# itz-sayak/C-Users-Sayakdutta-Self-Supervised-Arbitrary-Scale-Point-Cloud-Upsampling-via-SNN

Measured on AMD Instinct MI355X. Metric: upsampled query-points/sec (kNN + fn fwd + rotate + fd fwd + displace), 4x scale, M=48 T=4, higher is better.
Workload: dtype f32 (GEMMs as 3 x f16 MFMA with f32 accumulation; outer kNN f64); 1 GPU; synthetic sphere N=5000 (seed 0), B=4096 grid queries per GPU per step, M=48, T=4, fn k=[24,18,12] emb 640, fd k=32 scales [8,16,32,48] emb 768, conditioned-random weights seed 0, in-patch kNN recomputed every batch; cloud_points=5000, neighbours=48, outer_knn=f64 brute force, parallelism=query shards x1

## Files before the change

c-users-sayakdutta-self-supervised-arbitrary-scale-point-cloud-upsampling-via-snn_amd/csrc/common.h:

```cpp
#pragma once
#include <hip/hip_runtime.h>
#include <stdint.h>
#include <stdio.h>
#include <string.h>
#include "../../include/sapcu.h"

namespace sapcu {

void set_error(const char* fmt, ...);

#define SAPCU_CHECK_ARG(cond, ...)                      \
    do {                                                \
        if (!(cond)) {                                  \
            ::sapcu::set_error(__VA_ARGS__);            \
            return SAPCU_ERR_ARG;                       \
        }                                               \
    } while (0)

#define SAPCU_CHECK_HIP(expr)                                                            \
    do {                                                                                 \
        hipError_t _e = (expr);                                                          \
        if (_e != hipSuccess) {                                                          \
            ::sapcu::set_error("%s failed: %s (%s:%d)", #expr, hipGetErrorString(_e),    \
                               __FILE__, __LINE__);                                      \
// ... 134 lines not shown
    g = g * 0.19947114020071633897f;
#else
    const f32x2 a = pk_fma(x * x, f32x2{-0.72134752044448170368f, -0.72134752044448170368f},
                           f32x2{-2.3257480647361593f, -2.3257480647361593f});
    g.x = __builtin_amdgcn_exp2f(a.x);
    g.y = __builtin_amdgcn_exp2f(a.y);
#endif
    e.x = __builtin_amdgcn_exp2f(b.x);
    e.y = __builtin_amdgcn_exp2f(b.y);
    const f32x2 den = e + 1.0f;
    s.x = __builtin_amdgcn_rcpf(den.x);
    s.y = __builtin_amdgcn_rcpf(den.y);
    return pk_fma(f32x2{0.5f, 0.5f}, s, g);
}

template <int H>
__device__ __forceinline__ void lif_selfloop_pairs(f32x2 (&v)[H], const NeuronP2 (&p)[H], int T) {
    f32x2 m[H], r[H], th[H], s[H];
#pragma unroll
    for (int u = 0; u < H; ++u) {
        m[u] = v[u];
        s[u] = soft_spike2(m[u] - p[u].theta0);
    }
    if (T > 1) {
#ifdef SAPCU_LIF_EXACT_ORDER
#pragma unroll
        for (int u = 0; u < H; ++u) {
            m[u] = m[u] * (1.0f - s[u]);
            r[u] = s[u];
            const f32x2 t0 = p[u].theta0 + p[u].adapt * s[u];
            th[u] = p[u].theta0 + (t0 - p[u].theta0) * 0.95f;
        }
// ... 13 lines not shown
        for (int u = 0; u < H; ++u) {
            const f32x2 mm = (m[u] * p[u].decay) * (1.0f - r[u]);
            s[u] = soft_spike2(mm - th[u]);
        }
#else
        f32x2 a95[H], thc[H];
        const f32x2 k95 = f32x2{0.95f, 0.95f};
#pragma unroll
        for (int u = 0; u < H; ++u) {
            a95[u] = p[u].adapt * 0.95f;
            thc[u] = p[u].theta0 * 0.05f;
            m[u] = pk_fma(-m[u], s[u], m[u]);
            r[u] = s[u];
            th[u] = pk_fma(p[u].theta0, k95, pk_fma(s[u], a95[u], thc[u]));
        }
        for (int t = 1; t < T - 1; ++t) {
#pragma unroll
            for (int u = 0; u < H; ++u) {
                const f32x2 md = m[u] * p[u].decay;
                const f32x2 mm = pk_fma(-md, r[u], md);
                const f32x2 sp = soft_spike2(mm - th[u]);
                m[u] = pk_fma(-mm, sp, mm);
                r[u] = pk_fma(r[u], p[u].rdecay, sp);
                th[u] = pk_fma(th[u], k95, pk_fma(sp, a95[u], thc[u]));
                s[u] = sp;
            }
        }
#pragma unroll
        for (int u = 0; u < H; ++u) {
            const f32x2 md = m[u] * p[u].decay;
            s[u] = soft_spike2(pk_fma(-md, r[u], md) - th[u]);
        }
#endif
    }
#pragma unroll
    for (int u = 0; u < H; ++u) v[u] = s[u];
}

template <int W>
__device__ __forceinline__ void lif_selfloop_n(float (&v)[W], const NeuronP& p, int T) {
    constexpr int H = (W + 1) / 2;
    f32x2 pv[H];
    NeuronP2 pp[H];
#pragma unroll
    for (int u = 0; u < H; ++u) {
        pv[u] = f32x2{v[2 * u], v[(2 * u + 1 < W) ? 2 * u + 1 : 2 * u]};
        pp[u] = NeuronP2{{p.decay, p.decay}, {p.adapt, p.adapt}, {p.rdecay, p.rdecay}, {p.theta0, p.theta0}};
    }
    lif_selfloop_pairs<H>(pv, pp, T);
#pragma unroll
    for (int u = 0; u < H; ++u) {
        v[2 * u] = pv[u].x;
        if (2 * u + 1 < W) v[2 * u + 1] = pv[u].y;
    }
}

__device__ __forceinline__ float lif_selfloop(float x, const NeuronP& p, int T) {
    float v[1] = {x};
    lif_selfloop_n<1>(v, p, T);
    return v[0];
}

struct NeuronS2 {
    f32x2 m, th, r;
// ... 208 lines not shown
```

c-users-sayakdutta-self-supervised-arbitrary-scale-point-cloud-upsampling-via-snn_amd/csrc/fn_edge_chain.hip:

```cpp
#include "common.h"
#include "gemm_epi.h"
#include "ops.h"

namespace sapcu {
typedef _Float16 half8 __attribute__((ext_vector_type(8)));

#ifndef SAPCU_CHAIN_LB128
#define SAPCU_CHAIN_LB128 3
#endif
#ifndef SAPCU_CHAIN_FCD_MFMA
#define SAPCU_CHAIN_FCD_MFMA(D) ((D) == 256)
#endif
template <int D> struct ChainShape {
    static constexpr int ROWS = D == 128 ? 96 : (D == 256 ? 128 : 64);
    static constexpr int RS = ROWS / 16;
    static constexpr int CB = D == 512 ? 2 : 1;
    static constexpr int CS = 2 * CB;
    static constexpr int NW = D / (32 * CB);
    static constexpr int PLANE = ROWS * 64;
    static constexpr int KSTEP = 2 * PLANE;
    static constexpr int LDS = ROWS * D * 4 + ROWS * 16 + ROWS * 8;
    static constexpr int US = 8;
};

template <int D, int KK> struct ChainSlots {
    static constexpr int GS = 4 * ChainShape<D>::RS;
// ... 5 lines not shown
        if (t < KK) return g;
        const int p = 4 + (g * SP + t - KK) / KK;
        return p < PPG ? p : -1;
    }
    static constexpr int nbr(int rs, int g, int e) {
        const int t = 4 * rs + e;
        return t < KK ? t : (g * SP + t - KK) % KK;
    }
    static constexpr int SP1 = SP > 0 ? SP : 1;
    static constexpr int ua_g(int n, int jj) { return (n * KK + jj) / SP1; }
    static constexpr int ua_rs(int n, int jj) { return (KK + (n * KK + jj) % SP1) >> 2; }
    static constexpr int ua_e(int n, int jj) { return (KK + (n * KK + jj) % SP1) & 3; }
};

__global__ __launch_bounds__(256) void edge_prep_kernel(const float* __restrict__ patch, const int32_t* __restrict__ idx,
                                                        int64_t rows, int m, int kk, int2* __restrict__ tab,
                                                        float4* __restrict__ pd) {
    const int64_t r = (int64_t)blockIdx.x * blockDim.x + threadIdx.x;
    if (r >= rows) return;
    const int64_t pt = r / kk;
    const int64_t nrow = (pt / m) * m + idx[r];
    tab[r] = make_int2((int)pt, (int)nrow);
    const float* pi = patch + pt * 3;
    const float* pj = patch + nrow * 3;
    pd[r] = make_float4(__fsub_rn(pi[0], pj[0]), __fsub_rn(pi[1], pj[1]), __fsub_rn(pi[2], pj[2]), 0.f);
}

__global__ __launch_bounds__(256) void pack_chain_weights_kernel(const _Float16* __restrict__ hi, const _Float16* __restrict__ lo,
                                                                 int d, _Float16* __restrict__ out) {
    const int64_t t = (int64_t)blockIdx.x * blockDim.x + threadIdx.x;
    const int nk32 = d / 32;
    const int64_t total = (int64_t)(d / 16) * nk32 * 2 * 64;
    if (t >= total) return;
    const int lane = (int)(t & 63);
    const int plane = (int)((t >> 6) & 1);
    const int64_t cs_s = t >> 7;
    const int s = (int)(cs_s % nk32), cs = (int)(cs_s / nk32);
    const _Float16* src = (plane ? lo : hi) + (int64_t)(16 * cs + (lane & 15)) * d + 32 * s + 8 * (lane >> 4);
    *reinterpret_cast<half8*>(out + t * 8) = *reinterpret_cast<const half8*>(src);
}
// ... 224 lines not shown
#pragma unroll
    for (int jj = 0; jj < KK; jj += 2) {
        const f32x2 w2 = f32x2{xs[jj], xs[jj + 1]} * inv2;
        out = __fmaf_rn(w2.x, ts[jj], out);
        out = __fmaf_rn(w2.y, ts[jj + 1], out);
    }
    return out;
}

template <int KK>
__device__ __forceinline__ float chain_softmax_agg(float (&xs)[KK], const float (&ts)[KK]) {
    const float den = chain_softmax_den<KK>(xs);
    return chain_softmax_out<KK>(xs, ts, den);
}

template <int D, int KK, bool O32, bool FILL, bool TRIM>
__device__ __forceinline__ void fn_edge_chain_body(const ChainArgs& a) {
    static_assert(!FILL || (D == 512 && KK == 12), "filled groups: d = 512, kk = 12");
    static_assert(ChainSlots<D, KK>::NUA == 0 || (ChainSlots<D, KK>::NUA == 1 && ChainSlots<D, KK>::SP == 4 && KK == 12) ||
                      (ChainSlots<D, KK>::NUA == 3 && ChainSlots<D, KK>::SP == 14 && KK == 18),
                  "the trimmed spare-slot sums are written for the slot layouts of d = 256 / kk = 18 and d = 512 / kk = 12");
    using S = ChainShape<D>;
    using M = ChainSlots<D, KK>;
    constexpr int CH_ROWS = S::ROWS, RS = S::RS, CS = S::CS, CH_PLANE = S::PLANE, CH_KSTEP = S::KSTEP;
    constexpr int PPG = M::PPG, NUA = M::NUA, SP = M::SP;
    constexpr int NUP = RS / 2;
    constexpr bool TRIM_FCD = TRIM && SAPCU_CHAIN_FCD_MFMA(D);
    extern __shared__ __attribute__((aligned(1024))) unsigned char smem[];
    unsigned char* X = smem;
    float* pdx = reinterpret_cast<float*>(smem + CH_ROWS * D * 4);
    float* pdy = pdx + CH_ROWS;
    float* pdz = pdy + CH_ROWS;
    int2* rinfo = reinterpret_cast<int2*>(smem + CH_ROWS * D * 4 + CH_ROWS * 16);

    const int tid = threadIdx.x;
    const int lane = tid & 63;
    const int w = __builtin_amdgcn_readfirstlane(tid >> 6);
    const int cs0 = w * CS;
    ChainLane<CS> L;
    L.c16 = lane & 15;
    L.g = lane >> 4;
    const bool g0 = (L.g & 1) != 0, g1 = (L.g & 2) != 0;
// ... 31 lines not shown
    f32x4 acc[RS][CS], pe[RS][CS];
    ChainW<CS> W;
    CHAIN_STAMP(0);
    if (tid < CH_ROWS) {
        const int rs = tid >> 4, sg = (tid >> 2) & 3, e = tid & 3, t = 4 * rs + e;
        int p, jj;
        if (t < KK) {
            p = sg;
            jj = t;
        } else {
            const int u = sg * SP + t - KK;
            p = 4 + u / KK;
            jj = u % KK;
        }
        const bool ok = p < npts;
        int64_t er = ok ? (pt0 + p) * KK + jj : pt0 * KK;
        if (FILL && p >= PPG && strad >= 0) er = strad * KK + 4 * spos + jj;
        const int2 t2 = a.tab[er];
        if (O32) reinterpret_cast<unsigned*>(rinfo)[tid] = (unsigned)t2.y * (unsigned)(a.ldq * 4);
        else rinfo[tid] = t2;
        const float4 dv = a.pd[er];
        pdx[tid] = dv.x;
        pdy[tid] = dv.y;
        pdz[tid] = dv.z;
        if (TRIM_FCD) pdz[CH_ROWS + tid] = 1.0f;
    }
    CHAIN_STAMP(1);
    lds_barrier();
    float pa[RS], wb[CS];
    auto fc_delta_unit = [&](int j, int up) {
#pragma unroll
        for (int hq = 0; hq < 2; ++hq)
            acc[2 * up + hq][j] = __builtin_amdgcn_mfma_f32_16x16x4f32(pa[2 * up + hq], wb[j], f32x4{-0.f, -0.f, -0.f, -0.f}, 0, 0, 0);
    };
    if (TRIM_FCD) {
#pragma unroll
// ... 23 lines not shown
            } else {
#pragma unroll
                for (int hq = 0; hq < 2; ++hq) {
                    const int r0 = 16 * (2 * up + hq) + rowg;
                    const float4 qx = *reinterpret_cast<const float4*>(pdx + r0), qy = *reinterpret_cast<const float4*>(pdy + r0),
                                 qz = *reinterpret_cast<const float4*>(pdz + r0);
                    const f32x2 wx2 = f32x2{wx, wx}, wy2 = f32x2{wy, wy}, wz2 = f32x2{wz, wz}, bd2 = f32x2{bd, bd};
                    const f32x2 ta = pk_fma(wz2, f32x2{qz.x, qz.y}, pk_fma(wy2, f32x2{qy.x, qy.y}, wx2 * f32x2{qx.x, qx.y})) + bd2;
                    const f32x2 tb = pk_fma(wz2, f32x2{qz.z, qz.w}, pk_fma(wy2, f32x2{qy.z, qy.w}, wx2 * f32x2{qx.z, qx.w})) + bd2;
                    v[4 * hq] = ta.x;
                    v[4 * hq + 1] = ta.y;
                    v[4 * hq + 2] = tb.x;
                    v[4 * hq + 3] = tb.y;
                }
            }
            lif_selfloop_n<8>(v, nd, a.T);
#pragma unroll
            for (int z = 0; z < 8; z += 2) chain_put2<CH_PLANE, CS>(X, L, j, 2 * up + (z >> 2), z & 3, v[z], v[z + 1]);
            __builtin_amdgcn_sched_barrier(0);
        }
    }
    CHAIN_STAMP(2);
    const half8* const wp1 = reinterpret_cast<const half8*>(a.w1p);
    const half8* const wp2 = reinterpret_cast<const half8*>(a.w2p);
    const half8* const wp3 = reinterpret_cast<const half8*>(a.w3p);
    float kq[2][8], vq[2][8];
    auto gather_kv = [&](int j, int up, float (&kd)[8], float (&vd)[8]) {
#pragma unroll
        for (int z = 0; z < 8; ++z) {
            const int row = 16 * (2 * up + (z >> 2)) + rowg + (z & 3);
            if (O32) {
// ... 25 lines not shown
        CHAIN_STAMP(4);
        lds_barrier();
        CHAIN_STAMP(5);
#pragma unroll
        for (int j = 0; j < CS; ++j) {
            const float b1 = a.b1[L.col[j]];
            const NeuronP n1 = chain_lif(a.lif1, D, L.col[j]);
            if (j + 1 < CS) load_q(j + 1, qa[(j + 1) & 1], qu[(j + 1) & 1], qs[(j + 1) & 1]);
#pragma unroll
            for (int up = 0; up < NUP; ++up) {
                const int u = j * NUP + up;
                if (up + 1 < NUP) gather_kv(j, up + 1, kq[(u + 1) & 1], vq[(u + 1) & 1]);
                else if (j + 1 < CS) gather_kv(j + 1, 0, kq[(u + 1) & 1], vq[(u + 1) & 1]);
                __builtin_amdgcn_sched_barrier(0);
                float v[8];
#pragma unroll
                for (int z = 0; z < 8; ++z) v[z] = __fmaf_rn(acc[2 * up + (z >> 2)][j][z & 3], 0.0625f, b1);
                lif_selfloop_n<8>(v, n1, a.T);
                __builtin_amdgcn_sched_barrier(0);
                float ain[8];
#pragma unroll
                for (int z = 0; z < 8; ++z) {
                    const int rs = 2 * up + (z >> 2), e = z & 3;
                    float qv;
                    if (4 * rs + e < KK) {
                        qv = qa[j & 1];
                    } else {
                        float c[4];
#pragma unroll
                        for (int sg = 0; sg < 4; ++sg) {
                            const int p = M::point(rs, sg, e);
                            c[sg] = p >= 4 ? qu[j & 1][p - 4 < NUA ? p - 4 : 0] : (FILL && p < 0 ? qs[j & 1] : qa[j & 1]);
                        }
                        qv = group_select(c[0], c[1], c[2], c[3], g0, g1);
                    }
                    ain[z] = __fadd_rn(__fsub_rn(qv, kq[u & 1][z]), v[z]);
                    pe[rs][j][e] = settle(__fadd_rn(vq[u & 1][z], v[z]));
                }
#pragma unroll
                for (int z = 0; z < 8; z += 2) chain_put2<CH_PLANE, CS>(X, L, j, 2 * up + (z >> 2), z & 3, ain[z], ain[z + 1]);
                __builtin_amdgcn_sched_barrier(0);
            }
        }
        CHAIN_STAMP(6);
        chain_w_prefetch<D>(wp2, cs0, lane, W);
    }
    lds_barrier();
    CHAIN_STAMP(7);
    {
        chain_gemm<D>(X, wp2, cs0, lane, W, acc);
        CHAIN_STAMP(8);
        lds_barrier();
        CHAIN_STAMP(9);
#pragma unroll
        for (int j = 0; j < CS; ++j) {
            const float b2 = a.b2[L.col[j]];
            const NeuronP n2 = chain_lif(a.lif2, D, L.col[j]);
#pragma unroll
            for (int up = 0; up < NUP; ++up) {
                float v[8];
#pragma unroll
                for (int z = 0; z < 8; ++z) v[z] = __fmaf_rn(acc[2 * up + (z >> 2)][j][z & 3], 0.0625f, b2);
                lif_selfloop_n<8>(v, n2, a.T);
#pragma unroll
                for (int z = 0; z < 8; z += 2) chain_put2<CH_PLANE, CS>(X, L, j, 2 * up + (z >> 2), z & 3, v[z], v[z + 1]);
                __builtin_amdgcn_sched_barrier(0);
            }
        }
        CHAIN_STAMP(10);
        chain_w_prefetch<D>(wp3, cs0, lane, W);
    }
    lds_barrier();
    CHAIN_STAMP(11);
    {
        chain_gemm<D>(X, wp3, cs0, lane, W, acc);
        CHAIN_STAMP(12);
        CHAIN_T0();
        auto scale_rows = [&](int j) {
// ... 217 lines not shown
            if ((NUA == 3 ? L.g > 0 : L.g == 2) && st_pt < npts) {
#pragma unroll
                for (int j = 0; j < CS; ++j) {
                    if (a.res_split) chain_store_split_nt(a.res, pt0 + st_pt, D, L.col[j], o_end[j]);
                    else __builtin_nontemporal_store(o_end[j], &a.res[(pt0 + st_pt) * D + L.col[j]]);
                }
            }
            CHAIN_TACC(t_spare);
#undef CHAIN_SX
#undef CHAIN_ST
        }
        CHAIN_STAMP_END();
    }
}

template <int D, int KK, bool O32, bool TRIM>
__global__ __launch_bounds__(ChainShape<D>::NW * 64, (D == 128 ? SAPCU_CHAIN_LB128 : 1)) void fn_edge_chain_kernel(const ChainArgs a) {
    fn_edge_chain_body<D, KK, O32, false, TRIM>(a);
}

template <bool O32, bool TRIM>
__global__ __launch_bounds__(ChainShape<512>::NW * 64, 1) void fn_edge_chain_fill_kernel(const ChainArgs a) {
    fn_edge_chain_body<512, 12, O32, true, TRIM>(a);
}

template <int KK>
__global__ __launch_bounds__(256) void fn_chain_straddler_kernel(const float* __restrict__ fx, const float* __restrict__ ft, int64_t nsuper,
                                                                 int d, float* __restrict__ res, int res_split) {
    const int64_t t = (int64_t)blockIdx.x * blockDim.x + threadIdx.x;
    if (t >= nsuper * d) return;
    const int64_t sgi = t / d;
    const int col = (int)(t - sgi * d);
    float xs[KK], ts[KK];
#pragma unroll
    for (int jj = 0; jj < KK; ++jj) {
        xs[jj] = __builtin_nontemporal_load(&fx[(sgi * KK + jj) * d + col]);
        ts[jj] = __builtin_nontemporal_load(&ft[(sgi * KK + jj) * d + col]);
    }
    const float out = chain_softmax_agg<KK>(xs, ts);
    const int64_t pt = 16 * sgi + 15;
    if (res_split) chain_store_split_nt(res, pt, d, col, out);
    else __builtin_nontemporal_store(out, &res[pt * d + col]);
}

template <int D, int KK, bool O32, bool TRIM>
static int launch_chain_t(const ChainArgs& a, hipStream_t st) {
    constexpr int lds = ChainShape<D>::LDS;
    static DeviceOnce lds_once;
    SAPCU_SET_MAX_LDS(lds_once, (&fn_edge_chain_kernel<D, KK, O32, TRIM>), lds);
    constexpr int PPG = ChainSlots<D, KK>::PPG;
    const int64_t ngroups = (a.P + PPG - 1) / PPG;
    const int64_t grid = ngroups < 8 ? ngroups : ((ngroups + 7) / 8) * 8;
    SAPCU_CHECK_ARG(grid < 0x7fffffffLL, "edge_chain: too many groups");
    hipLaunchKernelGGL((fn_edge_chain_kernel<D, KK, O32, TRIM>), dim3((unsigned)grid), dim3(ChainShape<D>::NW * 64), lds, st, a);
    SAPCU_CHECK_LAUNCH();
    return SAPCU_OK;
}

template <int D, int KK>
static int launch_chain_plain(const ChainArgs& a, bool o32, hipStream_t st) {
    if (a.trim) return o32 ? launch_chain_t<D, KK, true, true>(a, st) : launch_chain_t<D, KK, false, true>(a, st);
    return o32 ? launch_chain_t<D, KK, true, false>(a, st) : launch_chain_t<D, KK, false, false>(a, st);
}

template <bool O32, bool TRIM>
static int launch_chain_fill_t(const ChainArgs& a, hipStream_t st) {
    constexpr int lds = ChainShape<512>::LDS, PPG = ChainSlots<512, 12>::PPG;
    static DeviceOnce lds_once;
    SAPCU_SET_MAX_LDS(lds_once, (&fn_edge_chain_fill_kernel<O32, TRIM>), lds);
    const int64_t nsuper = a.P / 16;
    const int64_t ngroups = 3 * nsuper + (a.P - 16 * nsuper + PPG - 1) / PPG;
    const int64_t grid = ngroups < 8 ? ngroups : ((ngroups + 7) / 8) * 8;
    SAPCU_CHECK_ARG(grid < 0x7fffffffLL, "edge_chain: too many groups");
    hipLaunchKernelGGL((fn_edge_chain_fill_kernel<O32, TRIM>), dim3((unsigned)grid), dim3(ChainShape<512>::NW * 64), lds, st, a);
    SAPCU_CHECK_LAUNCH();
    hipLaunchKernelGGL((fn_chain_straddler_kernel<12>), dim3((unsigned)((nsuper * 512 + 255) / 256)), dim3(256), 0, st, a.fill_x, a.fill_t,
                       nsuper, 512, a.res, a.res_split);
    SAPCU_CHECK_LAUNCH();
    return SAPCU_OK;
}

bool fn_edge_chain_ok(int d, int kk) { return (d == 128 && kk == 24) || (d == 256 && kk == 18) || (d == 512 && kk == 12); }

int launch_fn_edge_chain(ChainArgs a, const float* patch, const int32_t* idx, int d, int kk, int2* tab, float4* pd,
                         hipStream_t st) {
    if (a.P == 0) return SAPCU_OK;
    SAPCU_CHECK_ARG(fn_edge_chain_ok(d, kk), "edge_chain: unsupported block shape d=%d kk=%d", d, kk);
    SAPCU_CHECK_ARG(a.P * (int64_t)kk < 0x7fffffffLL && a.P * (int64_t)(a.ldq) < (1LL << 40), "edge_chain: too many rows");
    const int64_t rows = a.P * kk;
    hipLaunchKernelGGL(edge_prep_kernel, dim3((unsigned)((rows + 255) / 256)), dim3(256), 0, st, patch, idx, rows, a.m, kk, tab, pd);
    SAPCU_CHECK_LAUNCH();
    a.tab = tab;
    a.pd = pd;
    const bool o32 = !a.wide_offsets && (uint64_t)a.P * (uint64_t)a.ldq * 4u + 3u * (uint64_t)d * 4u < (1ull << 32) && a.ldq > 0;
    if (d == 128) return launch_chain_plain<128, 24>(a, o32, st);
    if (d == 256) return launch_chain_plain<256, 18>(a, o32, st);
    if (a.fill_x && a.fill_t && a.P >= 16) {
        if (a.trim) return o32 ? launch_chain_fill_t<true, true>(a, st) : launch_chain_fill_t<false, true>(a, st);
        return o32 ? launch_chain_fill_t<true, false>(a, st) : launch_chain_fill_t<false, false>(a, st);
    }
    return launch_chain_plain<512, 12>(a, o32, st);
}

int launch_pack_chain_weights(const void* w16_hi, const void* w16_lo, int d, void* out, hipStream_t st) {
    const int64_t total = (int64_t)(d / 16) * (d / 32) * 2 * 64;
    hipLaunchKernelGGL(pack_chain_weights_kernel, dim3((unsigned)((total + 255) / 256)), dim3(256), 0, st,
                       (const _Float16*)w16_hi, (const _Float16*)w16_lo, d, (_Float16*)out);
    SAPCU_CHECK_LAUNCH();
    return SAPCU_OK;
}

}
```

c-users-sayakdutta-self-supervised-arbitrary-scale-point-cloud-upsampling-via-snn_amd/csrc/model.hip:

```cpp
#include <stdarg.h>
#include <stdlib.h>

#include <new>
#include <vector>

#include "common.h"
#include "ops.h"

namespace sapcu {

static thread_local char g_err[512] = "";

void set_error(const char* fmt, ...) {
    va_list ap;
    va_start(ap, fmt);
    vsnprintf(g_err, sizeof(g_err), fmt, ap);
    va_end(ap);
}

enum FnSlot {
    FN_STEM_W = 0, FN_STEM_B, FN_STEM_LIF,
    FN_BLK0 = 3,
    FN_FINAL_W = FN_BLK0 + 63, FN_FINAL_B, FN_FINAL_LIF,
    FN_FCOUT_W, FN_FCOUT_B,
// ... 42 lines not shown
    int32_t* ks_dev = nullptr;
    int* gate_dev = nullptr;
    bool sf16 = true;
    void* w16_hi = nullptr;
    void* w16_lo = nullptr;
    void* chain_w = nullptr;
    int* ovf_dev = nullptr;
    int emb = 0, T = 0, heads = 0;
    int64_t chunk = 0;
    int64_t ws_budget = 0;
    bool opt_bt = true;
    bool opt_chain = true;
    bool opt_chain_wide = false;
    bool opt_chain_fill = true;
    bool opt_chain_trim = true;
    bool opt_shortk = true;
    bool opt_fn_maxfuse = true;
    bool opt_fn_fold_out = true;
    bool opt_fd_maxfuse = true;
    bool opt_fd_split = true;
    bool opt_fd_fused = true;
    bool opt_fd_x0 = true;
    void* fde_w = nullptr;
    int64_t fde_off[5] = {0, 0, 0, 0, 0};
    float* fde_nprm = nullptr;
    float* blob = nullptr;
    int64_t blob_floats = 0;
    int64_t fold_w[3] = {0, 0, 0}, fold_b[3] = {0, 0, 0};
    std::vector<int64_t> dir;
    const float* p(int slot) const { return blob + dir[slot]; }
// ... 28 lines not shown
    }
}

static bool env_is(const char* name, const char* value) {
    const char* e = getenv(name);
    return e && strcmp(e, value) == 0;
}

static void read_env_switches(sapcu_model* m) {
    m->sf16 = !env_is("SAPCU_GEMM", "f32");
    m->opt_bt = !env_is("SAPCU_BT", "0");
    m->opt_chain = !env_is("SAPCU_CHAIN", "0");
    m->opt_chain_wide = env_is("SAPCU_CHAIN", "wide");
    m->opt_chain_fill = !env_is("SAPCU_CHAIN_FILL", "0");
    m->opt_chain_trim = !env_is("SAPCU_CHAIN_TRIM", "0");
    m->opt_shortk = !env_is("SAPCU_SHORTK", "0");
    m->opt_fn_maxfuse = !env_is("SAPCU_FN_MAXFUSE", "0");
    m->opt_fn_fold_out = !env_is("SAPCU_FN_FOLD_OUT", "0");
    m->opt_fd_maxfuse = !env_is("SAPCU_FD_MAXFUSE", "0");
    m->opt_fd_split = !env_is("SAPCU_FD_SPLIT", "0");
    m->opt_fd_fused = !env_is("SAPCU_FD_FUSED", "0");
    m->opt_fd_x0 = !env_is("SAPCU_FD_X0", "0");
    const char* ce = getenv("SAPCU_CHUNK");
    m->chunk = ce ? atoll(ce) : 0;
    if (m->chunk < 0) m->chunk = 0;
    const char* be = getenv("SAPCU_WS_BUDGET_MB");
    m->ws_budget = (be ? atoll(be) : 20480) * (int64_t)(1 << 20);
    if (m->ws_budget < (int64_t)(64 << 20)) m->ws_budget = (int64_t)(64 << 20);
}

// ... 144 lines not shown
    return w;
}

static int64_t chain_w_off(int l, int q) {
    int64_t off = 0;
    for (int i = 0; i < l; ++i) off += (int64_t)3 * 2 * (128 << i) * (128 << i);
    return off + (int64_t)q * 2 * (128 << l) * (128 << l);
}

struct FnEdge {
    const float* pc;
    int64_t P;
    int mp, l, d, kk, sb, SP;
    float sqrt_hd;
    int64_t b1_floats;
};

static int fn_edge_chain_fused(const sapcu_model* m, const FnWs& W, const FnEdge& e, hipStream_t st) {
    const int d = e.d, sb = e.sb;
    ChainArgs ca;
    memset(&ca, 0, sizeof(ca));
    ca.P = e.P; ca.m = e.mp; ca.qkv = W.QKV; ca.ldq = 3 * d;
    ca.wd = m->p(sb + B_DELTA_W); ca.bd = m->p(sb + B_DELTA_B); ca.lifd = m->p(sb + B_DELTA_LIF);
    const _Float16* cw = (const _Float16*)m->chain_w;
    ca.w1p = cw + chain_w_off(e.l, 0); ca.b1 = m->p(sb + B_DELTA2_B); ca.lif1 = m->p(sb + B_DELTA2_LIF);
    ca.w2p = cw + chain_w_off(e.l, 1); ca.b2 = m->p(sb + B_GAMMA_B); ca.lif2 = m->p(sb + B_GAMMA_LIF);
    ca.w3p = cw + chain_w_off(e.l, 2); ca.b3 = m->p(sb + B_GAMMA2_B);
    ca.inv_sqrt_hd = 1.0f / e.sqrt_hd;
    ca.res = W.RES; ca.res_split = e.SP; ca.T = 4; ca.wide_offsets = m->opt_chain_wide ? 1 : 0;
    ca.trim = m->opt_chain_trim ? 1 : 0;
    if (m->opt_chain_fill && d == 512 && e.kk == 12) {
        const int64_t need = (e.P / 16) * 12 * 512;
        if (need > 0 && need <= e.P * 512 && need <= e.b1_floats) {
            ca.fill_x = W.X;
            ca.fill_t = W.B1;
        }
    }
    return launch_fn_edge_chain(ca, e.pc, W.idx[e.l], d, e.kk, W.tab, W.pdiff, st);
}

static int fn_edge_chain_unfused(const sapcu_model* m, const FnWs& W, const FnEdge& e, hipStream_t st) {
    const int d = e.d, kk = e.kk, sb = e.sb, SP = e.SP;
    const int64_t R = e.P * kk;
    const int32_t* idx = W.idx[e.l];
    SAPCU_TRY(launch_fn_pe1(e.pc, idx, R, e.mp, kk, d, m->p(sb + B_DELTA_W), m->p(sb + B_DELTA_B), m->p(sb + B_DELTA_LIF), 4, W.B1, SP,
                            st));
    {
        GemmArgs g;
        memset(&g, 0, sizeof(g));
        g.a = W.B1; g.r = R; g.k = d; g.lda = d; g.w = m->p(sb + B_DELTA2_W); g.n = d;
        g.bias = m->p(sb + B_DELTA2_B); g.c = W.B2; g.ldc = d; g.epi = EPI_LIF_ATTN;
        g.lif = m->p(sb + B_DELTA2_LIF); g.lif_T = 4; g.c2 = W.B3;
        g.q = W.QKV; g.kf = W.QKV + d; g.ldq = 3 * d; g.tab = W.tab;
// ... 8 lines not shown
}

static int fn_forward(const sapcu_model* m, const float* patch, int64_t b, int mp, const int32_t* knn_in,
                      int32_t* knn_out, float* normals, void* ws, int64_t ws_bytes, void* const* taps,
                      hipStream_t st) {
    const FnPlan pl = fn_plan(m, b, mp);
    const FnWs W = fn_ws_layout(ws_align256(ws), m, pl, mp);
    if (ws_bytes < (int64_t)W.bytes + 256) {
        set_error("fn_forward: workspace %lld B < required %lld B", (long long)ws_bytes, (long long)W.bytes + 256);
        return SAPCU_ERR_WORKSPACE;
    }
    int64_t tab_off[3];
    tab_off[0] = 0;
    tab_off[1] = b * mp * pl.kk[0];
    tab_off[2] = tab_off[1] + b * mp * pl.kk[1];

    for (int64_t s = 0; s < b; s += pl.cb) {
        const int64_t cb = (b - s) < pl.cb ? (b - s) : pl.cb;
        const int64_t P = cb * mp;
        const float* pc = patch + s * mp * 3;

        if (!knn_in) SAPCU_TRY(launch_patch_knn_multi(pc, cb, (int64_t)mp * 3, mp, 3, 3, 3, pl.kk, W.idx, st));
        for (int l = 0; l < 3; ++l) {
            const int64_t cnt = P * pl.kk[l];
            if (knn_in)
                SAPCU_CHECK_HIP(hipMemcpyAsync(W.idx[l], knn_in + tab_off[l] + s * mp * pl.kk[l], cnt * 4,
                                               hipMemcpyDeviceToDevice, st));
            if (knn_out)
                SAPCU_CHECK_HIP(hipMemcpyAsync(knn_out + tab_off[l] + s * mp * pl.kk[l], W.idx[l], cnt * 4,
                                               hipMemcpyDeviceToDevice, st));
        }
        SAPCU_TRY(launch_fn_stem(pc, P, m->p(FN_STEM_W), m->p(FN_STEM_B), m->p(FN_STEM_LIF), m->T, W.feat0, st));
        SAPCU_TRY(tap_copy(taps, SAPCU_FN_TAP_STEM, s * mp * 64 * 4, W.feat0, P * 64 * 4, st));

        const float* fin = W.feat0;
        int ldin = 64;
        for (int l = 0; l < 3; ++l) {
            const int d = 128 << l;
            const int sb = FN_BLK0 + l * B_SLOTS;
            const int SP = m->sf16 ? 1 : 0;
            float* const out = W.cat + 64 * l;
            SAPCU_TRY(gemm(m, fin, P, 64, ldin, m->p(sb + B_FC1_W), d, m->p(sb + B_FC1_B), W.X, d, EPI_LIF, st,
                           m->p(sb + B_SNN1), 4, nullptr, 0, SP << 1));
            SAPCU_TRY(gemm(m, W.X, P, d, d, m->p(sb + B_QKV_W), 3 * d, m->p(sb + B_QKV_B), W.QKV, 3 * d, EPI_LIF, st,
                           m->p(sb + B_QKV_LIF), 4, nullptr, 0, SP));
            const FnEdge e{pc, P, mp, l, d, pl.kk[l], sb, SP, (float)sqrt((double)(d / m->heads)), pl.edge_floats};
            SAPCU_TRY(fn_block_fused(m, l, mp) ? fn_edge_chain_fused(m, W, e, st) : fn_edge_chain_unfused(m, W, e, st));
            if (m->opt_fn_fold_out) {
                SAPCU_TRY(gemm(m, W.RES, P, d, d, m->blob + m->fold_w[l], 64, m->blob + m->fold_b[l], out, 192, EPI_RESID, st,
                               nullptr, 0, fin, ldin, SP));
            } else {
                SAPCU_TRY(gemm(m, W.RES, P, d, d, m->p(sb + B_OUT_W), d, m->p(sb + B_OUT_B), W.X, d, EPI_BIAS, st, nullptr, 0, nullptr,
                               0, SP | (SP << 1)));
                SAPCU_TRY(gemm(m, W.X, P, d, d, m->p(sb + B_FC2_W), 64, m->p(sb + B_FC2_B), out, 192, EPI_RESID, st,
                               nullptr, 0, fin, ldin, SP));
            }
            if (taps && taps[SAPCU_FN_TAP_BLOCK1 + l]) {
                SAPCU_CHECK_HIP(hipMemcpy2DAsync((char*)taps[SAPCU_FN_TAP_BLOCK1 + l] + s * mp * 64 * 4, 64 * 4,
                                                 out, 192 * 4, 64 * 4, (size_t)P, hipMemcpyDeviceToDevice, st));
            }
            fin = out;
// ... 492 lines not shown
    for (int q = 0; q < 3; ++q) {
        GemmArgs g;
        memset(&g, 0, sizeof(g));
        SAPCU_TRY(split_into_ws(ws[q], (int64_t)d * d, W.split[q], g, st));
        SAPCU_TRY(launch_pack_chain_weights(g.w16_hi, g.w16_lo, d, W.packed[q], st));
    }
    ChainArgs ca;
    memset(&ca, 0, sizeof(ca));
    ca.P = points; ca.m = m_pts; ca.qkv = qkv; ca.ldq = 3 * d;
    ca.wd = w_delta; ca.bd = b_delta; ca.lifd = lif_delta;
    ca.w1p = W.packed[0]; ca.b1 = b1; ca.lif1 = lif1;
    ca.w2p = W.packed[1]; ca.b2 = b2; ca.lif2 = lif2;
    ca.w3p = W.packed[2]; ca.b3 = b3;
    ca.inv_sqrt_hd = 1.0f / (float)sqrt((double)(d / heads));
    ca.res = res_out; ca.res_split = 0; ca.T = lif_steps;
    ca.trim = 1;
#ifdef CHAIN_STAMPS
    {
        const int64_t sbytes = (points / 4 + 1) * 16 * 8;
        const int64_t off = (need + 255) / 256 * 256;
        if (workspace_bytes >= off + sbytes + 256) ca.stamps = (unsigned long long*)((char*)ws_align256(workspace) + off);
        if (env_is("SAPCU_CHAIN_TRIM", "0")) ca.trim = 0;
    }
#endif
    return launch_fn_edge_chain(ca, patch, idx, d, kk, W.tab, W.pd, st);
}

int sapcu_model_create(int kind, const int32_t* hp, int n_hp, const float* blob, int64_t blob_floats,
                       const int64_t* dir_host, int n_dir, sapcu_model_t* out) {
    SAPCU_CHECK_ARG(hp && blob && dir_host && out && blob_floats > 0, "model_create: null pointer");
    sapcu_model* m = new (std::nothrow) sapcu_model();
    SAPCU_CHECK_ARG(m != nullptr, "model_create: out of host memory");
    m->kind = kind;
    read_env_switches(m);
    int rc = SAPCU_OK;
    if (kind == SAPCU_KIND_FN) {
        if (n_hp != 6 || n_dir != FN_SLOTS) {
            set_error("model_create(fn): need 6 hparams and %d slots (got %d, %d)", (int)FN_SLOTS, n_hp, n_dir);
            rc = SAPCU_ERR_ARG;
        } else {
// ... 217 lines not shown
```

c-users-sayakdutta-self-supervised-arbitrary-scale-point-cloud-upsampling-via-snn_amd/csrc/ops.h:

```cpp
#pragma once
#include "common.h"

namespace sapcu {

int launch_patch_knn_strided(const float* feat, int64_t b, int64_t pstride, int m, int c, int ld, int k,
                             int32_t* idx, hipStream_t st);
int launch_patch_knn_multi(const float* feat, int64_t b, int64_t pstride, int m, int c, int ld, int ntab,
                           const int* ks, int32_t* const* idx, hipStream_t st);
int launch_patch_knn(const float* feat, int64_t b, int m, int c, int ld, int k, int32_t* idx, hipStream_t st);
int launch_neuron_selfloop(const float* x, int64_t rows, int ch, int T, const float* md, const float* ta,
                           const float* rd, const float* tb, const float* dT, const float* rh, float* so, float* mo,
                           float* to, float* ro, hipStream_t st);
int launch_neuron_drive(const float* x, int64_t rows, int ch, int T, const float* md, const float* ta, const float* rd, const float* tb,
                        const float* dT, const float* rh, int pairv, float* so, float* mo, float* to, float* ro, int* gate, hipStream_t st);
int launch_fn_stem(const float* patch, int64_t rows, const float* w, const float* bias, const float* lif, int T,
                   float* out, hipStream_t st);
int launch_fn_pe1(const float* patch, const int32_t* idx, int64_t rows, int m, int kk, int d, const float* w,
                  const float* bias, const float* lif, int T, float* out, int split, hipStream_t st);
struct ChainArgs {
    int64_t P;
    int m;
    const int2* tab;
    const float4* pd;
    const float* qkv;
    int ldq;
    const float* wd;
    const float* bd;
    const float* lifd;
    const _Float16* w1p;
    const float* b1;
    const float* lif1;
    const _Float16* w2p;
    const float* b2;
    const float* lif2;
    const _Float16* w3p;
    const float* b3;
    float inv_sqrt_hd;
    float* res;
    int res_split;
    int T;
    int wide_offsets;
    float* fill_x;
    float* fill_t;
    int trim;
#ifdef CHAIN_STAMPS
    unsigned long long* stamps;
#endif
};
bool fn_edge_chain_ok(int d, int kk);
int launch_fn_edge_chain(ChainArgs a, const float* patch, const int32_t* idx, int d, int kk, int2* tab_ws, float4* pd_ws,
                         hipStream_t st);
int launch_pack_chain_weights(const void* w16_hi, const void* w16_lo, int d, void* out, hipStream_t st);
int launch_edge_table(const int32_t* idx, int64_t rows, int m, int kk, int2* tab, hipStream_t st);
int launch_fn_softmax_agg(const float* a, const float* pe, const float* v, int ldv, const int32_t* idx, int64_t pts,
                          int m, int kk, int d, float sqrt_hd, float* res, int split, hipStream_t st);
int launch_decode_max_keys(const unsigned* keys, int64_t count, float* out, hipStream_t st);
int launch_rowgroup_max(const float* in, int64_t groups, int m, int c, float* out, hipStream_t st);
int launch_fn_tail(const float* h, int64_t b, int kdim, const float* w, const float* bias, const float* lnw,
                   const float* lnb, float* logits, float* normals, hipStream_t st);
int launch_to_split_rows(const float* in, int64_t rows, int k, int ld_in, float* out, int ld_out, hipStream_t st);
int launch_l2_normalize3(const float* in, float* out, int64_t b, hipStream_t st);
int launch_fd_edge0(const float* patch, const int32_t* idx, int kmax, int64_t pts, int m, int nscale,
                    const int32_t* ks_dev, const float* w, const float* bias, float* out, hipStream_t st);
int launch_fd_neuron(bool eif, int mode, const float* in, int ldi, const int32_t* idx, int kk, int m,
                     const float* shift, int64_t pts, int C, const float* prm, int T, float* spk, int ldo, int coff,
// ... 58 lines not shown
```

Measured before the change: 134,800 query-points/s.

## Merge edge tables into one float4 record, share across FN blocks, specialize T=4

New measurement: 135,600 query-points/s (median of 6 runs). No clear change (+0.6%).

```diff
diff --git a/c-users-sayakdutta-self-supervised-arbitrary-scale-point-cloud-upsampling-via-snn_amd/csrc/common.h b/c-users-sayakdutta-self-supervised-arbitrary-scale-point-cloud-upsampling-via-snn_amd/csrc/common.h
--- a/c-users-sayakdutta-self-supervised-arbitrary-scale-point-cloud-upsampling-via-snn_amd/csrc/common.h
+++ b/c-users-sayakdutta-self-supervised-arbitrary-scale-point-cloud-upsampling-via-snn_amd/csrc/common.h
@@ -172,8 +172,9 @@
     return pk_fma(f32x2{0.5f, 0.5f}, s, g);
 }
 
-template <int H>
-__device__ __forceinline__ void lif_selfloop_pairs(f32x2 (&v)[H], const NeuronP2 (&p)[H], int T) {
+template <int H, int TC = 0>
+__device__ __forceinline__ void lif_selfloop_pairs(f32x2 (&v)[H], const NeuronP2 (&p)[H], int T_rt) {
+    const int T = TC > 0 ? TC : T_rt;
     f32x2 m[H], r[H], th[H], s[H];
 #pragma unroll
     for (int u = 0; u < H; ++u) {
@@ -217,7 +218,7 @@
             r[u] = s[u];
             th[u] = pk_fma(p[u].theta0, k95, pk_fma(s[u], a95[u], thc[u]));
         }
-        for (int t = 1; t < T - 1; ++t) {
+        auto mid = [&]() {
 #pragma unroll
             for (int u = 0; u < H; ++u) {
                 const f32x2 md = m[u] * p[u].decay;
@@ -228,6 +229,12 @@
                 th[u] = pk_fma(th[u], k95, pk_fma(sp, a95[u], thc[u]));
                 s[u] = sp;
             }
+        };
+        if constexpr (TC > 0) {
+#pragma unroll
+            for (int t = 1; t < TC - 1; ++t) mid();
+        } else {
+            for (int t = 1; t < T - 1; ++t) mid();
         }
 #pragma unroll
         for (int u = 0; u < H; ++u) {
@@ -240,7 +247,7 @@
     for (int u = 0; u < H; ++u) v[u] = s[u];
 }
 
-template <int W>
+template <int W, int TC = 0>
 __device__ __forceinline__ void lif_selfloop_n(float (&v)[W], const NeuronP& p, int T) {
     constexpr int H = (W + 1) / 2;
     f32x2 pv[H];
@@ -250,7 +257,7 @@
         pv[u] = f32x2{v[2 * u], v[(2 * u + 1 < W) ? 2 * u + 1 : 2 * u]};
         pp[u] = NeuronP2{{p.decay, p.decay}, {p.adapt, p.adapt}, {p.rdecay, p.rdecay}, {p.theta0, p.theta0}};
     }
-    lif_selfloop_pairs<H>(pv, pp, T);
+    lif_selfloop_pairs<H, TC>(pv, pp, T);
 #pragma unroll
     for (int u = 0; u < H; ++u) {
         v[2 * u] = pv[u].x;
diff --git a/c-users-sayakdutta-self-supervised-arbitrary-scale-point-cloud-upsampling-via-snn_amd/csrc/fn_edge_chain.hip b/c-users-sayakdutta-self-supervised-arbitrary-scale-point-cloud-upsampling-via-snn_amd/csrc/fn_edge_chain.hip
--- a/c-users-sayakdutta-self-supervised-arbitrary-scale-point-cloud-upsampling-via-snn_amd/csrc/fn_edge_chain.hip
+++ b/c-users-sayakdutta-self-supervised-arbitrary-scale-point-cloud-upsampling-via-snn_amd/csrc/fn_edge_chain.hip
@@ -10,6 +10,12 @@
 #endif
 #ifndef SAPCU_CHAIN_FCD_MFMA
 #define SAPCU_CHAIN_FCD_MFMA(D) ((D) == 256)
+#endif
+#ifndef SAPCU_CHAIN_PK
+#define SAPCU_CHAIN_PK(D) ((D) == 512)
+#endif
+#ifndef SAPCU_CHAIN_T4
+#define SAPCU_CHAIN_T4(D) true
 #endif
 template <int D> struct ChainShape {
     static constexpr int ROWS = D == 128 ? 96 : (D == 256 ? 128 : 64);
@@ -45,16 +51,14 @@
 };
 
 __global__ __launch_bounds__(256) void edge_prep_kernel(const float* __restrict__ patch, const int32_t* __restrict__ idx,
-                                                        int64_t rows, int m, int kk, int2* __restrict__ tab,
-                                                        float4* __restrict__ pd) {
+                                                        int64_t rows, int m, int kk, float4* __restrict__ rec) {
     const int64_t r = (int64_t)blockIdx.x * blockDim.x + threadIdx.x;
     if (r >= rows) return;
     const int64_t pt = r / kk;
     const int64_t nrow = (pt / m) * m + idx[r];
-    tab[r] = make_int2((int)pt, (int)nrow);
     const float* pi = patch + pt * 3;
     const float* pj = patch + nrow * 3;
-    pd[r] = make_float4(__fsub_rn(pi[0], pj[0]), __fsub_rn(pi[1], pj[1]), __fsub_rn(pi[2], pj[2]), 0.f);
+    rec[r] = make_float4(__fsub_rn(pi[0], pj[0]), __fsub_rn(pi[1], pj[1]), __fsub_rn(pi[2], pj[2]), __int_as_float((int)nrow));
 }
 
 __global__ __launch_bounds__(256) void pack_chain_weights_kernel(const _Float16* __restrict__ hi, const _Float16* __restrict__ lo,
@@ -309,7 +313,24 @@
     return chain_softmax_out<KK>(xs, ts, den);
 }
 
-template <int D, int KK, bool O32, bool FILL, bool TRIM>
+template <bool PK>
+__device__ __forceinline__ void chain_scale_bias(const f32x4& q0, const f32x4& q1, float b, float (&v)[8]) {
+    if constexpr (PK) {
+        const f32x2 k16 = f32x2{0.0625f, 0.0625f}, b2 = f32x2{b, b};
+#pragma unroll
+        for (int z = 0; z < 8; z += 2) {
+            const f32x4& q = z < 4 ? q0 : q1;
+            const f32x2 s2 = pk_fma(f32x2{q[z & 3], q[(z & 3) + 1]}, k16, b2);
+            v[z] = s2.x;
+            v[z + 1] = s2.y;
+        }
+    } else {
+#pragma unroll
+        for (int z = 0; z < 8; ++z) v[z] = __fmaf_rn((z < 4 ? q0 : q1)[z & 3], 0.0625f, b);
+    }
+}
+
+template <int D, int KK, bool O32, bool FILL, bool TRIM, int TC>
 __device__ __forceinline__ void fn_edge_chain_body(const ChainArgs& a) {
     static_assert(!FILL || (D == 512 && KK == 12), "filled groups: d = 512, kk = 12");
     static_assert(ChainSlots<D, KK>::NUA == 0 || (ChainSlots<D, KK>::NUA == 1 && ChainSlots<D, KK>::SP == 4 && KK == 12) ||
@@ -321,6 +342,7 @@
     constexpr int PPG = M::PPG, NUA = M::NUA, SP = M::SP;
     constexpr int NUP = RS / 2;
     constexpr bool TRIM_FCD = TRIM && SAPCU_CHAIN_FCD_MFMA(D);
+    constexpr bool PK = TRIM && SAPCU_CHAIN_PK(D);
     extern __shared__ __attribute__((aligned(1024))) unsigned char smem[];
     unsigned char* X = smem;
     float* pdx = reinterpret_cast<float*>(smem + CH_ROWS * D * 4);
@@ -382,12 +404,13 @@
             jj = u % KK;
         }
         const bool ok = p < npts;
-        int64_t er = ok ? (pt0 + p) * KK + jj : pt0 * KK;
-        if (FILL && p >= PPG && strad >= 0) er = strad * KK + 4 * spos + jj;
-        const int2 t2 = a.tab[er];
-        if (O32) reinterpret_cast<unsigned*>(rinfo)[tid] = (unsigned)t2.y * (unsigned)(a.ldq * 4);
-        else rinfo[tid] = t2;
-        const float4 dv = a.pd[er];
+        const int64_t ks = a.rec_stride;
+        int64_t er = ok ? (pt0 + p) * ks + jj : pt0 * ks;
+        if (FILL && p >= PPG && strad >= 0) er = strad * ks + 4 * spos + jj;
+        const float4 dv = a.rec[er];
+        const int nrow = __float_as_int(dv.w);
+        if (O32) reinterpret_cast<unsigned*>(rinfo)[tid] = (unsigned)nrow * (unsigned)(a.ldq * 4);
+        else rinfo[tid] = make_int2(0, nrow);
         pdx[tid] = dv.x;
         pdy[tid] = dv.y;
         pdz[tid] = dv.z;
@@ -441,7 +464,7 @@
                     v[4 * hq + 3] = tb.y;
                 }
             }
-            lif_selfloop_n<8>(v, nd, a.T);
+            lif_selfloop_n<8, TC>(v, nd, a.T);
 #pragma unroll
             for (int z = 0; z < 8; z += 2) chain_put2<CH_PLANE, CS>(X, L, j, 2 * up + (z >> 2), z & 3, v[z], v[z + 1]);
             __builtin_amdgcn_sched_barrier(0);
@@ -497,28 +520,53 @@
                 else if (j + 1 < CS) gather_kv(j + 1, 0, kq[(u + 1) & 1], vq[(u + 1) & 1]);
                 __builtin_amdgcn_sched_barrier(0);
                 float v[8];
-#pragma unroll
-                for (int z = 0; z < 8; ++z) v[z] = __fmaf_rn(acc[2 * up + (z >> 2)][j][z & 3], 0.0625f, b1);
-                lif_selfloop_n<8>(v, n1, a.T);
+                chain_scale_bias<PK>(acc[2 * up][j], acc[2 * up + 1][j], b1, v);
+                lif_selfloop_n<8, TC>(v, n1, a.T);
                 __builtin_amdgcn_sched_barrier(0);
+                auto q_of = [&](int rs, int e) -> float {
+                    if (4 * rs + e < KK) return qa[j & 1];
+                    int cls[4];
+#pragma unroll
+                    for (int sg = 0; sg < 4; ++sg) {
+                        const int p = M::point(rs, sg, e);
+                        cls[sg] = p >= 4 ? 1 + (p - 4 < NUA ? p - 4 : 0) : (FILL && p < 0 ? 9 : 0);
+                    }
+                    auto val = [&](int c) { return c == 0 ? qa[j & 1] : (c == 9 ? qs[j & 1] : qu[j & 1][c >= 1 && c <= NUA ? c - 1 : 0]); };
+                    int second = -1;
+                    bool two = true;
+#pragma unroll
+                    for (int sg = 1; sg < 4; ++sg) {
+                        if (cls[sg] == cls[0] || cls[sg] == second) continue;
+                        if (second < 0) second = cls[sg];
+                        else two = false;
+                    }
+                    if (second < 0) return val(cls[0]);
+                    if (PK && two) {
+                        const bool in2 = (cls[1] == second && L.g == 1) || (cls[2] == second && L.g == 2) || (cls[3] == second && L.g == 3);
+                        return in2 ? val(second) : val(cls[0]);
+                    }
+                    return group_select(val(cls[0]), val(cls[1]), val(cls[2]), val(cls[3]), g0, g1);
+                };
                 float ain[8];
-#pragma unroll
-                for (int z = 0; z < 8; ++z) {
-                    const int rs = 2 * up + (z >> 2), e = z & 3;
-                    float qv;
-                    if (4 * rs + e < KK) {
-                        qv = qa[j & 1];
-                    } else {
-                        float c[4];
-#pragma unroll
-                        for (int sg = 0; sg < 4; ++sg) {
-                            const int p = M::point(rs, sg, e);
-                            c[sg] = p >= 4 ? qu[j & 1][p - 4 < NUA ? p - 4 : 0] : (FILL && p < 0 ? qs[j & 1] : qa[j & 1]);
-                        }
-                        qv = group_select(c[0], c[1], c[2], c[3], g0, g1);
-                    }
-                    ain[z] = __fadd_rn(__fsub_rn(qv, kq[u & 1][z]), v[z]);
-                    pe[rs][j][e] = settle(__fadd_rn(vq[u & 1][z], v[z]));
+                if constexpr (PK) {
+#pragma unroll
+                    for (int z = 0; z < 8; z += 2) {
+                        const int rs = 2 * up + (z >> 2), e = z & 3;
+                        const f32x2 v2 = f32x2{v[z], v[z + 1]};
+                        const f32x2 a2 = (f32x2{q_of(rs, e), q_of(rs, e + 1)} - f32x2{kq[u & 1][z], kq[u & 1][z + 1]}) + v2;
+                        const f32x2 t2 = f32x2{vq[u & 1][z], vq[u & 1][z + 1]} + v2;
+                        ain[z] = a2.x;
+                        ain[z + 1] = a2.y;
+                        pe[rs][j][e] = settle(t2.x);
+                        pe[rs][j][e + 1] = settle(t2.y);
+                    }
+                } else {
+#pragma unroll
+                    for (int z = 0; z < 8; ++z) {
+                        const int rs = 2 * up + (z >> 2), e = z & 3;
+                        ain[z] = __fadd_rn(__fsub_rn(q_of(rs, e), kq[u & 1][z]), v[z]);
+                        pe[rs][j][e] = settle(__fadd_rn(vq[u & 1][z], v[z]));
+                    }
                 }
 #pragma unroll
                 for (int z = 0; z < 8; z += 2) chain_put2<CH_PLANE, CS>(X, L, j, 2 * up + (z >> 2), z & 3, ain[z], ain[z + 1]);
@@ -542,9 +590,8 @@
 #pragma unroll
             for (int up = 0; up < NUP; ++up) {
                 float v[8];
-#pragma unroll
-                for (int z = 0; z < 8; ++z) v[z] = __fmaf_rn(acc[2 * up + (z >> 2)][j][z & 3], 0.0625f, b2);
-                lif_selfloop_n<8>(v, n2, a.T);
+                chain_scale_bias<PK>(acc[2 * up][j], acc[2 * up + 1][j], b2, v);
+                lif_selfloop_n<8, TC>(v, n2, a.T);
 #pragma unroll
                 for (int z = 0; z < 8; z += 2) chain_put2<CH_PLANE, CS>(X, L, j, 2 * up + (z >> 2), z & 3, v[z], v[z + 1]);
                 __builtin_amdgcn_sched_barrier(0);
@@ -792,14 +839,14 @@
     }
 }
 
-template <int D, int KK, bool O32, bool TRIM>
+template <int D, int KK, bool O32, bool TRIM, int TC>
 __global__ __launch_bounds__(ChainShape<D>::NW * 64, (D == 128 ? SAPCU_CHAIN_LB128 : 1)) void fn_edge_chain_kernel(const ChainArgs a) {
-    fn_edge_chain_body<D, KK, O32, false, TRIM>(a);
-}
-
-template <bool O32, bool TRIM>
+    fn_edge_chain_body<D, KK, O32, false, TRIM, TC>(a);
+}
+
+template <bool O32, bool TRIM, int TC>
 __global__ __launch_bounds__(ChainShape<512>::NW * 64, 1) void fn_edge_chain_fill_kernel(const ChainArgs a) {
-    fn_edge_chain_body<512, 12, O32, true, TRIM>(a);
+    fn_edge_chain_body<512, 12, O32, true, TRIM, TC>(a);
 }
 
 template <int KK>
@@ -821,36 +868,39 @@
     else __builtin_nontemporal_store(out, &res[pt * d + col]);
 }
 
-template <int D, int KK, bool O32, bool TRIM>
+template <int D, int KK, bool O32, bool TRIM, int TC>
 static int launch_chain_t(const ChainArgs& a, hipStream_t st) {
     constexpr int lds = ChainShape<D>::LDS;
     static DeviceOnce lds_once;
-    SAPCU_SET_MAX_LDS(lds_once, (&fn_edge_chain_kernel<D, KK, O32, TRIM>), lds);
+    SAPCU_SET_MAX_LDS(lds_once, (&fn_edge_chain_kernel<D, KK, O32, TRIM, TC>), lds);
     constexpr int PPG = ChainSlots<D, KK>::PPG;
     const int64_t ngroups = (a.P + PPG - 1) / PPG;
     const int64_t grid = ngroups < 8 ? ngroups : ((ngroups + 7) / 8) * 8;
     SAPCU_CHECK_ARG(grid < 0x7fffffffLL, "edge_chain: too many groups");
-    hipLaunchKernelGGL((fn_edge_chain_kernel<D, KK, O32, TRIM>), dim3((unsigned)grid), dim3(ChainShape<D>::NW * 64), lds, st, a);
+    hipLaunchKernelGGL((fn_edge_chain_kernel<D, KK, O32, TRIM, TC>), dim3((unsigned)grid), dim3(ChainShape<D>::NW * 64), lds, st, a);
     SAPCU_CHECK_LAUNCH();
     return SAPCU_OK;
 }
 
 template <int D, int KK>
 static int launch_chain_plain(const ChainArgs& a, bool o32, hipStream_t st) {
-    if (a.trim) return o32 ? launch_chain_t<D, KK, true, true>(a, st) : launch_chain_t<D, KK, false, true>(a, st);
-    return o32 ? launch_chain_t<D, KK, true, false>(a, st) : launch_chain_t<D, KK, false, false>(a, st);
-}
-
-template <bool O32, bool TRIM>
+    if constexpr (SAPCU_CHAIN_T4(D)) {
+        if (a.trim && a.T == 4) return o32 ? launch_chain_t<D, KK, true, true, 4>(a, st) : launch_chain_t<D, KK, false, true, 4>(a, st);
+    }
+    if (a.trim) return o32 ? launch_chain_t<D, KK, true, true, 0>(a, st) : launch_chain_t<D, KK, false, true, 0>(a, st);
+    return o32 ? launch_chain_t<D, KK, true, false, 0>(a, st) : launch_chain_t<D, KK, false, false, 0>(a, st);
+}
+
+template <bool O32, bool TRIM, int TC>
 static int launch_chain_fill_t(const ChainArgs& a, hipStream_t st) {
     constexpr int lds = ChainShape<512>::LDS, PPG = ChainSlots<512, 12>::PPG;
     static DeviceOnce lds_once;
-    SAPCU_SET_MAX_LDS(lds_once, (&fn_edge_chain_fill_kernel<O32, TRIM>), lds);
+    SAPCU_SET_MAX_LDS(lds_once, (&fn_edge_chain_fill_kernel<O32, TRIM, TC>), lds);
     const int64_t nsuper = a.P / 16;
     const int64_t ngroups = 3 * nsuper + (a.P - 16 * nsuper + PPG - 1) / PPG;
     const int64_t grid = ngroups < 8 ? ngroups : ((ngroups + 7) / 8) * 8;
     SAPCU_CHECK_ARG(grid < 0x7fffffffLL, "edge_chain: too many groups");
-    hipLaunchKernelGGL((fn_edge_chain_fill_kernel<O32, TRIM>), dim3((unsigned)grid), dim3(ChainShape<512>::NW * 64), lds, st, a);
+    hipLaunchKernelGGL((fn_edge_chain_fill_kernel<O32, TRIM, TC>), dim3((unsigned)grid), dim3(ChainShape<512>::NW * 64), lds, st, a);
     SAPCU_CHECK_LAUNCH();
     hipLaunchKernelGGL((fn_chain_straddler_kernel<12>), dim3((unsigned)((nsuper * 512 + 255) / 256)), dim3(256), 0, st, a.fill_x, a.fill_t,
                        nsuper, 512, a.res, a.res_split);
@@ -860,22 +910,28 @@
 
 bool fn_edge_chain_ok(int d, int kk) { return (d == 128 && kk == 24) || (d == 256 && kk == 18) || (d == 512 && kk == 12); }
 
-int launch_fn_edge_chain(ChainArgs a, const float* patch, const int32_t* idx, int d, int kk, int2* tab, float4* pd,
+int launch_fn_edge_chain(ChainArgs a, const float* patch, const int32_t* idx, int d, int kk, float4* rec, int rec_stride,
                          hipStream_t st) {
     if (a.P == 0) return SAPCU_OK;
     SAPCU_CHECK_ARG(fn_edge_chain_ok(d, kk), "edge_chain: unsupported block shape d=%d kk=%d", d, kk);
-    SAPCU_CHECK_ARG(a.P * (int64_t)kk < 0x7fffffffLL && a.P * (int64_t)(a.ldq) < (1LL << 40), "edge_chain: too many rows");
-    const int64_t rows = a.P * kk;
-    hipLaunchKernelGGL(edge_prep_kernel, dim3((unsigned)((rows + 255) / 256)), dim3(256), 0, st, patch, idx, rows, a.m, kk, tab, pd);
-    SAPCU_CHECK_LAUNCH();
-    a.tab = tab;
-    a.pd = pd;
+    SAPCU_CHECK_ARG(rec && rec_stride >= kk && rec_stride <= a.m, "edge_chain: bad record table (stride %d, kk %d)", rec_stride, kk);
+    SAPCU_CHECK_ARG(a.P * (int64_t)rec_stride < 0x7fffffffLL && a.P * (int64_t)(a.ldq) < (1LL << 40), "edge_chain: too many rows");
+    if (idx) {
+        const int64_t rows = a.P * rec_stride;
+        hipLaunchKernelGGL(edge_prep_kernel, dim3((unsigned)((rows + 255) / 256)), dim3(256), 0, st, patch, idx, rows, a.m, rec_stride, rec);
+        SAPCU_CHECK_LAUNCH();
+    }
+    a.rec = rec;
+    a.rec_stride = rec_stride;
     const bool o32 = !a.wide_offsets && (uint64_t)a.P * (uint64_t)a.ldq * 4u + 3u * (uint64_t)d * 4u < (1ull << 32) && a.ldq > 0;
     if (d == 128) return launch_chain_plain<128, 24>(a, o32, st);
     if (d == 256) return launch_chain_plain<256, 18>(a, o32, st);
     if (a.fill_x && a.fill_t && a.P >= 16) {
-        if (a.trim) return o32 ? launch_chain_fill_t<true, true>(a, st) : launch_chain_fill_t<false, true>(a, st);
-        return o32 ? launch_chain_fill_t<true, false>(a, st) : launch_chain_fill_t<false, false>(a, st);
+        if constexpr (SAPCU_CHAIN_T4(512)) {
+            if (a.trim && a.T == 4) return o32 ? launch_chain_fill_t<true, true, 4>(a, st) : launch_chain_fill_t<false, true, 4>(a, st);
+        }
+        if (a.trim) return o32 ? launch_chain_fill_t<true, true, 0>(a, st) : launch_chain_fill_t<false, true, 0>(a, st);
+        return o32 ? launch_chain_fill_t<true, false, 0>(a, st) : launch_chain_fill_t<false, false, 0>(a, st);
     }
     return launch_chain_plain<512, 12>(a, o32, st);
 }
diff --git a/c-users-sayakdutta-self-supervised-arbitrary-scale-point-cloud-upsampling-via-snn_amd/csrc/model.hip b/c-users-sayakdutta-self-supervised-arbitrary-scale-point-cloud-upsampling-via-snn_amd/csrc/model.hip
--- a/c-users-sayakdutta-self-supervised-arbitrary-scale-point-cloud-upsampling-via-snn_amd/csrc/model.hip
+++ b/c-users-sayakdutta-self-supervised-arbitrary-scale-point-cloud-upsampling-via-snn_amd/csrc/model.hip
@@ -80,6 +80,7 @@
     bool opt_chain_wide = false;
     bool opt_chain_fill = true;
     bool opt_chain_trim = true;
+    bool opt_chain_tab = true;
     bool opt_shortk = true;
     bool opt_fn_maxfuse = true;
     bool opt_fn_fold_out = true;
@@ -138,6 +139,7 @@
     m->opt_chain_wide = env_is("SAPCU_CHAIN", "wide");
     m->opt_chain_fill = !env_is("SAPCU_CHAIN_FILL", "0");
     m->opt_chain_trim = !env_is("SAPCU_CHAIN_TRIM", "0");
+    m->opt_chain_tab = !env_is("SAPCU_CHAIN_TAB", "0");
     m->opt_shortk = !env_is("SAPCU_SHORTK", "0");
     m->opt_fn_maxfuse = !env_is("SAPCU_FN_MAXFUSE", "0");
     m->opt_fn_fold_out = !env_is("SAPCU_FN_FOLD_OUT", "0");
@@ -312,7 +314,16 @@
     int mp, l, d, kk, sb, SP;
     float sqrt_hd;
     int64_t b1_floats;
+    const int32_t* rec_idx;
+    int rec_stride;
 };
+
+static bool fn_shared_records(const sapcu_model* m, const FnPlan& pl, int mp, bool forced_tables) {
+    if (!m->opt_chain_tab || forced_tables) return false;
+    for (int l = 0; l < 3; ++l)
+        if (!fn_block_fused(m, l, mp) || pl.kk[l] != m->kv[l]) return false;
+    return pl.kk[0] >= pl.kk[1] && pl.kk[1] >= pl.kk[2];
+}
 
 static int fn_edge_chain_fused(const sapcu_model* m, const FnWs& W, const FnEdge& e, hipStream_t st) {
     const int d = e.d, sb = e.sb;
@@ -334,7 +345,7 @@
             ca.fill_t = W.B1;
         }
     }
-    return launch_fn_edge_chain(ca, e.pc, W.idx[e.l], d, e.kk, W.tab, W.pdiff, st);
+    return launch_fn_edge_chain(ca, e.pc, e.rec_idx, d, e.kk, W.pdiff, e.rec_stride, st);
 }
 
 static int fn_edge_chain_unfused(const sapcu_model* m, const FnWs& W, const FnEdge& e, hipStream_t st) {
@@ -373,6 +384,7 @@
     tab_off[0] = 0;
     tab_off[1] = b * mp * pl.kk[0];
     tab_off[2] = tab_off[1] + b * mp * pl.kk[1];
+    const bool shared_rec = fn_shared_records(m, pl, mp, knn_in != nullptr);
 
     for (int64_t s = 0; s < b; s += pl.cb) {
         const int64_t cb = (b - s) < pl.cb ? (b - s) : pl.cb;
@@ -403,7 +415,8 @@
                            m->p(sb + B_SNN1), 4, nullptr, 0, SP << 1));
             SAPCU_TRY(gemm(m, W.X, P, d, d, m->p(sb + B_QKV_W), 3 * d, m->p(sb + B_QKV_B), W.QKV, 3 * d, EPI_LIF, st,
                            m->p(sb + B_QKV_LIF), 4, nullptr, 0, SP));
-            const FnEdge e{pc, P, mp, l, d, pl.kk[l], sb, SP, (float)sqrt((double)(d / m->heads)), pl.edge_floats};
+            const FnEdge e{pc, P, mp, l, d, pl.kk[l], sb, SP, (float)sqrt((double)(d / m->heads)), pl.edge_floats,
+                           shared_rec ? (l == 0 ? W.idx[0] : nullptr) : W.idx[l], shared_rec ? pl.kk[0] : pl.kk[l]};
             SAPCU_TRY(fn_block_fused(m, l, mp) ? fn_edge_chain_fused(m, W, e, st) : fn_edge_chain_unfused(m, W, e, st));
             if (m->opt_fn_fold_out) {
                 SAPCU_TRY(gemm(m, W.RES, P, d, d, m->blob + m->fold_w[l], 64, m->blob + m->fold_b[l], out, 192, EPI_RESID, st,
@@ -926,16 +939,15 @@
     ca.w3p = W.packed[2]; ca.b3 = b3;
     ca.inv_sqrt_hd = 1.0f / (float)sqrt((double)(d / heads));
     ca.res = res_out; ca.res_split = 0; ca.T = lif_steps;
-    ca.trim = 1;
+    ca.trim = env_is("SAPCU_CHAIN_TRIM", "0") ? 0 : 1;
 #ifdef CHAIN_STAMPS
     {
         const int64_t sbytes = (points / 4 + 1) * 16 * 8;
         const int64_t off = (need + 255) / 256 * 256;
         if (workspace_bytes >= off + sbytes + 256) ca.stamps = (unsigned long long*)((char*)ws_align256(workspace) + off);
-        if (env_is("SAPCU_CHAIN_TRIM", "0")) ca.trim = 0;
     }
 #endif
-    return launch_fn_edge_chain(ca, patch, idx, d, kk, W.tab, W.pd, st);
+    return launch_fn_edge_chain(ca, patch, idx, d, kk, W.pd, kk, st);
 }
 
 int sapcu_model_create(int kind, const int32_t* hp, int n_hp, const float* blob, int64_t blob_floats,
diff --git a/c-users-sayakdutta-self-supervised-arbitrary-scale-point-cloud-upsampling-via-snn_amd/csrc/ops.h b/c-users-sayakdutta-self-supervised-arbitrary-scale-point-cloud-upsampling-via-snn_amd/csrc/ops.h
--- a/c-users-sayakdutta-self-supervised-arbitrary-scale-point-cloud-upsampling-via-snn_amd/csrc/ops.h
+++ b/c-users-sayakdutta-self-supervised-arbitrary-scale-point-cloud-upsampling-via-snn_amd/csrc/ops.h
@@ -20,8 +20,8 @@
 struct ChainArgs {
     int64_t P;
     int m;
-    const int2* tab;
-    const float4* pd;
+    const float4* rec;
+    int rec_stride;
     const float* qkv;
     int ldq;
     const float* wd;
@@ -48,7 +48,7 @@
 #endif
 };
 bool fn_edge_chain_ok(int d, int kk);
-int launch_fn_edge_chain(ChainArgs a, const float* patch, const int32_t* idx, int d, int kk, int2* tab_ws, float4* pd_ws,
+int launch_fn_edge_chain(ChainArgs a, const float* patch, const int32_t* idx, int d, int kk, float4* rec_ws, int rec_stride,
                          hipStream_t st);
 int launch_pack_chain_weights(const void* w16_hi, const void* w16_lo, int d, void* out, hipStream_t st);
 int launch_edge_table(const int32_t* idx, int64_t rows, int m, int kk, int2* tab, hipStream_t st);
```
